# Tongji-MIC-Lab/TDVC

Measured on AMD Instinct MI355X. Metric: 1080p P-frames/sec (encode + reconstruct, lambda=2048 config), higher is better.
Workload: dtype f16; 1 GPU; 1x 1920x1080 (padded 1088x1920) 7-frame synthetic GOP (seed 1234), batch 1, P-frames coded in GOP order; gop=7, batch=1, parallelism=gop-sharded x1, weights=closed-form filler (no checkpoint ships)

## Files before the change

### include/tdvc_hip.h

```cpp
#ifndef TDVC_HIP_H
#define TDVC_HIP_H

#include <stdint.h>

#ifdef __cplusplus
extern "C" {
#endif

#define TDVC_OK 0
#define TDVC_EINVAL (-1)
#define TDVC_ENOSUP (-2)

typedef struct {
  void* p;
  int32_t N, H, W, C;
  int64_t sn;
  int32_t sp;
  int32_t dtype;
} tdvc_fmap;

enum { TDVC_F16 = 0, TDVC_F32 = 1 };
enum { TDVC_ACT_NONE = 0, TDVC_ACT_RELU = 1, TDVC_ACT_LRELU = 2, TDVC_ACT_CLAMP01 = 3, TDVC_ACT_SIGMOID = 4 };
enum { TDVC_GDN_NONE = 0, TDVC_GDN_FWD = 1, TDVC_GDN_INV = 2 };
enum { TDVC_OUT_NHWC = 0,
// ... 36 lines not shown
int tdvc_last_launch_predicated(void);
#define TDVC_MAX_PREDICATE_IMAGES 4
int tdvc_set_predicate_images(const int* flags, int n);
int tdvc_frame_changed(const tdvc_fmap* cur, tdvc_fmap* cache, int* flag, void* stream);
int tdvc_frames_changed(const tdvc_fmap* cur, tdvc_fmap* cache, int* flags, unsigned force_mask, void* stream);


int tdvc_conv_plan(int cin, int kh, int kw, int stride);
int64_t tdvc_conv_packed_bytes(int cout, int cin, int ntaps, int ck);
int tdvc_pack_conv_weights(const float* w_oihw, int cout, int cin_real, int cin, int kh, int kw,
                           int ntaps, const int8_t* tap_dy, const int8_t* tap_dx, int ck, uint16_t* dst);
int tdvc_conv2d(const tdvc_conv_desc* d, void* stream);
int tdvc_conv_chan_sum_rows(const tdvc_conv_desc* d);
int tdvc_conv_flow_supported(const tdvc_conv_desc* d);
const char* tdvc_conv_select(const tdvc_conv_desc* d);
int tdvc_conv2d_f32(const tdvc_conv_desc* d, void* stream);

typedef struct {
  tdvc_fmap x, y;
  const void* w;
  const float* bias;
  int32_t act1; float slope1;
  int32_t act2; float slope2;
  int32_t add_input;
  tdvc_fmap res2;
} tdvc_conv_pair_desc;
int64_t tdvc_conv_pair_packed_bytes(void);
int tdvc_pack_conv_pair_weights(const float* w1_oihw, const float* w2_oihw, uint16_t* dst);
int tdvc_conv_pair_supported(const tdvc_conv_pair_desc* d);
int tdvc_conv_pair(const tdvc_conv_pair_desc* d, void* stream);
// ... 256 lines not shown
```

### tdvc_amd/_lib.py

```python
from __future__ import annotations

import ctypes as C
import os

_HERE = os.path.dirname(os.path.abspath(__file__))
LIB_PATH = os.path.join(_HERE, "libtdvc_hip.so")

MAX_TAPS = 49
F16, F32 = 0, 1
ACT_NONE, ACT_RELU, ACT_LRELU, ACT_CLAMP01, ACT_SIGMOID = 0, 1, 2, 3, 4
GDN_NONE, GDN_FWD, GDN_INV = 0, 1, 2
OUT_NHWC, OUT_SHUFFLE2, OUT_NCHW_F32 = 0, 1, 2


class FMapDesc(C.Structure):
    _fields_ = [("p", C.c_void_p), ("N", C.c_int32), ("H", C.c_int32), ("W", C.c_int32), ("C", C.c_int32),
                ("sn", C.c_int64), ("sp", C.c_int32), ("dtype", C.c_int32)]


class ConvDesc(C.Structure):
    _fields_ = [("x", FMapDesc), ("y", FMapDesc), ("w", C.c_void_p), ("bias", C.c_void_p),
                ("cout", C.c_int32), ("ntaps", C.c_int32),
                ("tap_dy", C.c_int8 * MAX_TAPS), ("tap_dx", C.c_int8 * MAX_TAPS),
                ("kh", C.c_int32), ("kw", C.c_int32), ("stride", C.c_int32), ("pad", C.c_int32),
# ... 45 lines not shown

class LanesEncDesc(C.Structure):
    _fields_ = [("symbols", _P), ("indexes", _P), ("B", C.c_int32), ("H", C.c_int32), ("W", C.c_int32), ("M", C.c_int32), ("pos", _P),
                ("npos", C.c_int32), ("L", C.c_int32), ("scratch", _P), ("lane_words", C.c_int64), ("scratch_cap_words", C.c_int64),
                ("out", _P), ("out_stride", C.c_int64), ("out_cap", C.c_int64), ("info", _P)]


_LOOP, _CDF, _CDFD, _ENC = C.POINTER(ArLoopDesc), C.POINTER(CdfTablesDesc), C.POINTER(CdfTablesDevDesc), C.POINTER(LanesEncDesc)
_i, _f, _i64 = C.c_int, C.c_float, C.c_int64

SIGNATURES = {
    "tdvc_abi_version": (_i, []),
    "tdvc_conv_chan_sum_rows": (_i, [C.POINTER(ConvDesc)]),
    "tdvc_conv_select": (C.c_char_p, [C.POINTER(ConvDesc)]),
    "tdvc_conv_flow_supported": (_i, [C.POINTER(ConvDesc)]),
    "tdvc_scale_act_res3": (_i, [_FM, _P, _i, _f, _FM, _f, _FM, _FM, _f, _FM, _P]),
    "tdvc_avgpool2_pyramid": (_i, [_FM, _FM, _FM, _FM, _P]),
    "tdvc_last_error": (C.c_char_p, []),
    "tdvc_last_conv_kernel": (C.c_char_p, []),
    "tdvc_prepare_device": (_i, []),
    "tdvc_set_predicate": (_i, [_P]),
    "tdvc_set_predicate_images": (_i, [_P, _i]),
    "tdvc_last_launch_predicated": (_i, []),
    "tdvc_frame_changed": (_i, [_FM, _FM, _P, _P]),
    "tdvc_frames_changed": (_i, [_FM, _FM, _P, C.c_uint, _P]),
    "tdvc_conv_plan": (_i, [_i, _i, _i, _i]),
    "tdvc_conv_packed_bytes": (_i64, [_i, _i, _i, _i]),
    "tdvc_pack_conv_weights": (_i, [_P, _i, _i, _i, _i, _i, _i, _P, _P, _i, _P]),
    "tdvc_conv2d": (_i, [C.POINTER(ConvDesc), _P]),
    "tdvc_conv2d_f32": (_i, [C.POINTER(ConvDesc), _P]),
# ... 131 lines not shown
```

### tdvc_amd/csrc/conv_dispatch.hip

```cpp
#include <stdlib.h>

#include "conv_common.h"

using convk::ConvParams;
bool conv_v2_eligible(const tdvc_conv_desc* d, int Ho, int Wo); int launch_conv_v2(const ConvParams& p, int cout_blocks, int N, hipStream_t st);
bool conv_v3_eligible(const tdvc_conv_desc* d, int Ho, int Wo); int launch_conv_v3(const ConvParams& p, int cout_blocks, int N, hipStream_t st);
bool conv_v5_eligible(const tdvc_conv_desc* d, int Ho, int Wo); int launch_conv_v5(const ConvParams& p, int cout_blocks, int N, hipStream_t st); int conv_v5_chan_sum_rows(int Ho, int Wo, int cout_blocks, int N);
bool conv_v7_eligible(const tdvc_conv_desc* d, const ConvParams& p, int Ho, int Wo); int launch_conv_v7(const ConvParams& p, int cout_blocks, int N, hipStream_t st);
bool conv_v9_eligible(const tdvc_conv_desc* d, int Ho, int Wo, bool v3_ok); int launch_conv_v9(const ConvParams& p, int ck8, int cout_tiles32, int N, hipStream_t st);
bool conv_v10_eligible(const tdvc_conv_desc* d, const ConvParams& p, int Ho, int Wo); int launch_conv_v10(const ConvParams& p, int cout_blocks, int N, hipStream_t st);
bool conv_v11_eligible(const tdvc_conv_desc* d, const ConvParams& p, int Ho, int Wo); int launch_conv_v11(const ConvParams& p, int cout_blocks, int N, hipStream_t st);
int conv_row_geometry(const tdvc_conv_desc* d, const ConvParams& p, int Ho, int Wo); int launch_conv_row(int geo, const ConvParams& p, int N, hipStream_t st);
bool conv_c8_eligible(const tdvc_conv_desc* d, const ConvParams& p, int Ho, int Wo); int launch_conv_c8(const ConvParams& p, int N, hipStream_t st);
bool conv_n16_eligible(const tdvc_conv_desc* d, int Ho, int Wo); int launch_conv_n16(const ConvParams& p, int N, hipStream_t st);
bool gdn128_eligible(const tdvc_conv_desc* d, const ConvParams& p, int Ho, int Wo); int launch_gdn128(const ConvParams& p, int N, hipStream_t st);
int conv_direct_lds_bytes(const tdvc_conv_desc* d);
int conv_cout_tiles(int cout);
int launch_conv_direct(const ConvParams& p, int ck8, int stride, int N, hipStream_t st);
int conv_f32_validate(const tdvc_conv_desc* d, int& Ho, int& Wo);

namespace {
const char* const kSwitchEnv[convk::SW_COUNT] = {nullptr, "TDVC_CONV_NO_V3", "TDVC_CONV_NO_V5", "TDVC_CONV_NO_V7", "TDVC_CONV_NO_V9", "TDVC_CONV_NO_V10",
                                                 "TDVC_CONV_NO_V11", "TDVC_CONV_NO_ROW", "TDVC_CONV_NO_C8", "TDVC_CONV_NO_N16", "TDVC_CONV_NO_GDN128", "TDVC_CONV_NO_HEAD3"};
int g_enabled[convk::SW_COUNT] = {1, 1, 1, 1, 1, 1, 1, 15, 1, 1, 1, 1};
// ... 59 lines not shown
  return launch_conv_v5(q, 1, k.N(), st);
}
bool row_eligible(Pick& k, const ConvParams& p) { return (k.geo = conv_row_geometry(k.d, p, k.Ho, k.Wo)) >= 0; }

constexpr char kNameV5[] = "conv_mfma_v5", kNameDirect[] = "conv_mfma<%d,%d,%d>";

const Entry kTable[] = {
    {"conv_mfma_v5(bcast)", convk::SW_V5, bcast_eligible, bcast_launch, [](const tdvc_conv_desc* d) { return d->bcast_T != 0; },
     "tdvc_conv2d: bcast_T needs a plain 1x1 / stride 1 conv to 64 channels of >= 8192 pixels, y (and res, the optional source of the slices) a 64-channel window of a buffer with >= 4 slices, bcast_T == 4"},
    {"conv_row(s2d)", convk::SW_ROW, [](Pick& k, const ConvParams& p) { return k.d->s2d && row_eligible(k, p); },
     [](const Pick& k, const ConvParams& p, hipStream_t st) { return launch_conv_row(k.geo, p, k.N(), st); }, nullptr, nullptr},
    {"conv_mfma_v3(s2d)", convk::SW_V3, [](Pick& k, const ConvParams&) { return k.d->s2d && conv_v3_eligible(k.d, k.Ho, k.Wo); },
     [](const Pick& k, const ConvParams& p, hipStream_t st) { return launch_conv_v3(p, k.cout_blocks(), k.N(), st); },
     [](const tdvc_conv_desc* d) { return d->s2d != 0; }, "tdvc_conv2d: s2d conv not eligible for the stage-pipelined kernel"},
    {"conv_mfma_v9", convk::SW_V9, [](Pick& k, const ConvParams&) { return conv_v9_eligible(k.d, k.Ho, k.Wo, v3_on_and_eligible(k)); },
     [](const Pick& k, const ConvParams& p, hipStream_t st) { return launch_conv_v9(p, k.ck8(), conv_cout_tiles(k.d->cout), k.N(), st); }, nullptr, nullptr},
    {"gdn128", convk::SW_GDN128, [](Pick& k, const ConvParams& p) { return gdn128_eligible(k.d, p, k.Ho, k.Wo); },
     [](const Pick& k, const ConvParams& p, hipStream_t st) { return launch_gdn128(p, k.N(), st); }, nullptr, nullptr},
    {kNameV5, convk::SW_V5, [](Pick& k, const ConvParams&) { return conv_v5_eligible(k.d, k.Ho, k.Wo); },
     [](const Pick& k, const ConvParams& p, hipStream_t st) { return launch_conv_v5(p, k.cout_blocks(), k.N(), st); }, nullptr, nullptr},
    {"conv_c8", convk::SW_C8, [](Pick& k, const ConvParams& p) { return conv_c8_eligible(k.d, p, k.Ho, k.Wo); },
     [](const Pick& k, const ConvParams& p, hipStream_t st) { return launch_conv_c8(p, k.N(), st); }, nullptr, nullptr},
    {"conv_n16", convk::SW_N16, [](Pick& k, const ConvParams&) { return conv_n16_eligible(k.d, k.Ho, k.Wo); },
     [](const Pick& k, const ConvParams& p, hipStream_t st) { return launch_conv_n16(p, k.N(), st); }, nullptr, nullptr},
    {"conv_row", convk::SW_ROW, row_eligible,
     [](const Pick& k, const ConvParams& p, hipStream_t st) { return launch_conv_row(k.geo, p, k.N(), st); }, nullptr, nullptr},
    {"conv_mfma_v10", convk::SW_V10, [](Pick& k, const ConvParams& p) { return conv_v10_eligible(k.d, p, k.Ho, k.Wo); },
     [](const Pick& k, const ConvParams& p, hipStream_t st) { return launch_conv_v10(p, k.cout_blocks(), k.N(), st); }, nullptr, nullptr},
    {"conv_mfma_v7", convk::SW_V7, [](Pick& k, const ConvParams& p) { return conv_v7_eligible(k.d, p, k.Ho, k.Wo); },
     [](const Pick& k, const ConvParams& p, hipStream_t st) { return launch_conv_v7(p, k.cout_blocks(), k.N(), st); }, nullptr, nullptr},
    {"conv_mfma_v11", convk::SW_V11, [](Pick& k, const ConvParams& p) { return conv_v11_eligible(k.d, p, k.Ho, k.Wo); },
// ... 142 lines not shown
  p.csum = d->chan_sum;
  if (!e) return TDVC_EINVAL;
  if (d->flow.p) {
    TDVC_CHECK(conv_flow_ok(d, e, p) && flow_map_ok(d, k.Ho, k.Wo), "%s", kFlowMsg);
    p.flow = to_dev(d->flow);
  }
  kernel_name(e, k, g_last_kernel);
  return e->launch(k, p, reinterpret_cast<hipStream_t>(stream));
}

}

void tdvc_conv_walk_advance(int launches) { g_walk_parity += (unsigned)launches; }

extern "C" void tdvc_debug_set_conv_walk(int mode) { g_walk_mode = mode; }
extern "C" int tdvc_conv2d(const tdvc_conv_desc* d, void* stream) { return conv2d_impl(d, stream, LAUNCH); }
extern "C" int tdvc_conv_chan_sum_rows(const tdvc_conv_desc* d) { return conv2d_impl(d, nullptr, QUERY_ROWS); }
extern "C" int tdvc_conv_flow_supported(const tdvc_conv_desc* d) { return conv2d_impl(d, nullptr, QUERY_FLOW); }
extern "C" const char* tdvc_last_conv_kernel(void) { return g_last_kernel; }

extern "C" const char* tdvc_conv_select(const tdvc_conv_desc* d) {
  static thread_local char name[48];
  if (!d) { tdvc_set_error("tdvc_conv_select: null descriptor"); return nullptr; }
  if (d->x.dtype == TDVC_F32) {
    int Ho, Wo;
    if (d->flow.p) { tdvc_set_error("%s", kFlowMsg); return nullptr; }
    return conv_f32_validate(d, Ho, Wo) == TDVC_OK ? "conv_f32" : nullptr;
  }
  ConvParams p;
  Pick k = {d, 0, 0, -1};
  if (prepare(d, p, k.Ho, k.Wo) != TDVC_OK) return nullptr;
  const Entry* e = select(k, p);
  if (!e) return nullptr;
  if (d->flow.p && !(conv_flow_ok(d, e, p) && flow_map_ok(d, k.Ho, k.Wo))) { tdvc_set_error("%s", kFlowMsg); return nullptr; }
// ... 4 lines not shown
```

### tdvc_amd/csrc/conv_mfma_v9.hip

```cpp
#include "conv_common.h"

using convk::ConvParams;

namespace {

template <int CK8, int NW9>
__global__ __launch_bounds__(NW9 * 64) void conv_mfma_v9_kernel(const ConvParams p, int total_px) {
  __shared__ float red[NW9][32][33];
  __shared__ int tdy[TDVC_MAX_TAPS], tdx[TDVC_MAX_TAPS];
  constexpr int CK = CK8 * 8;
  const int tid = threadIdx.x, lane = tid & 63, wave = tid >> 6;
  const int hh = lane >> 5, r = lane & 31;
  const int ct = blockIdx.y;
  if (tid < p.ntaps) { tdy[tid] = p.tap_dy[tid]; tdx[tid] = p.tap_dx[tid]; }
  __syncthreads();

  const int px = blockIdx.x * 32 + r;
  const bool pv = px < total_px;
  const int pxc = pv ? px : 0;
  const int hw = p.Ho * p.Wo;
  const int n = pxc / hw, rem = pxc - n * hw;
  const int oy = rem / p.Wo, ox = rem - oy * p.Wo;
  const int iy0 = oy * p.in_stride - p.pad, ix0 = ox * p.in_stride - p.pad;
  const half_t* xn = p.x + (long)n * p.x_sn;

  const int T = p.nchunks * p.steps;
  const int g0 = (int)((long)T * wave / NW9), g1 = (int)((long)T * (wave + 1) / NW9);
  const half_t* wp = p.w + ((long)ct * T) * 512 + lane * 8;

  f32x16 acc;
#pragma unroll
  for (int i = 0; i < 16; ++i) acc[i] = 0.f;
  half8 zero8;
#pragma unroll
  for (int q = 0; q < 8; ++q) zero8[q] = (half_t)0.f;

  for (int g4 = g0; g4 < g1; g4 += 4) {
    half8 a[4], b[4];
    bool ok[4];
#pragma unroll
    for (int u = 0; u < 4; ++u) {
      const int g = min(g4 + u, g1 - 1);
      const int ch = g / p.steps, s = g - ch * p.steps;
      int tap, cofs;
      if constexpr (CK8 == 1) {
        tap = min(2 * s + hh, p.ntaps - 1);
        cofs = ch * 8;
      } else {
        constexpr int H2 = CK8 / 2;
        tap = s / H2;
        cofs = ch * CK + (s - tap * H2) * 16 + hh * 8;
      }
      const int iy = iy0 + tdy[tap], ix = ix0 + tdx[tap];
      ok[u] = pv && g4 + u < g1 && iy >= 0 && iy < p.H && ix >= 0 && ix < p.W && cofs < p.Cin;
      const int iyc = min(max(iy, 0), p.H - 1), ixc = min(max(ix, 0), p.W - 1), cc = min(cofs, p.Cin - 8);
      b[u] = *reinterpret_cast<const half8*>(xn + ((long)iyc * p.W + ixc) * p.x_sp + cc);
      a[u] = *reinterpret_cast<const half8*>(wp + (long)g * 512);
    }
#pragma unroll
    for (int u = 0; u < 4; ++u) {
      half8 bv = ok[u] ? b[u] : zero8;
      if (p.square) bv = bv * bv;
      acc = __builtin_amdgcn_mfma_f32_32x32x16_f16(a[u], bv, acc, 0, 0, 0);
    }
  }

#pragma unroll
  for (int i = 0; i < 16; ++i) red[wave][(i & 3) + 8 * (i >> 2) + 4 * hh][r] = acc[i];
  __syncthreads();
  for (int it = tid; it < 256; it += NW9 * 64) {
    const int pl = it & 31, grp = it >> 5;
    const int q = blockIdx.x * 32 + pl;
    if (q < total_px) {
      float v[4];
#pragma unroll
      for (int i = 0; i < 4; ++i) {
        float s = 0.f;
#pragma unroll
        for (int w = 0; w < NW9; ++w) s += red[w][4 * grp + i][pl];
        v[i] = s;
      }
      const int qn = q / hw, qr = q - qn * hw;
      const int qy = qr / p.Wo, qx = qr - qy * p.Wo;
      convk::epilogue4(p, qn, qy, qx, ct * 32 + 4 * grp, v);
    }
  }
}

}

bool conv_v9_eligible(const tdvc_conv_desc* d, int Ho, int Wo, bool v3_ok) {
  if (d->s2d) return false;
  const long px = (long)Ho * Wo * d->x.N;
  static const long maxpx = getenv("TDVC_V9_MAX_PX") ? atol(getenv("TDVC_V9_MAX_PX")) : convk::LARGE_MAP_PIXELS;
  static const long minpx = getenv("TDVC_V9_MIN_PX") ? atol(getenv("TDVC_V9_MIN_PX")) : 0;
  const long ksteps = (long)((d->x.C + d->ck - 1) / d->ck) * ((d->ntaps * (d->ck / 8) + 1) / 2);
  if (v3_ok && px * d->cout > convk::conv_v9_work_limit()) return false;
  return px <= maxpx && px >= minpx && ksteps >= 4 && (d->x.C % 8) == 0;
}

template <int CK8>
static void launch_v9_nw(const ConvParams& p, dim3 grid, int total, hipStream_t st) {
  const int T = p.nchunks * p.steps;
  if (T >= 32) hipLaunchKernelGGL((conv_mfma_v9_kernel<CK8, 8>), grid, dim3(512), 0, st, p, total);
  else if (T >= 16) hipLaunchKernelGGL((conv_mfma_v9_kernel<CK8, 4>), grid, dim3(256), 0, st, p, total);
  else if (T >= 8) hipLaunchKernelGGL((conv_mfma_v9_kernel<CK8, 2>), grid, dim3(128), 0, st, p, total);
  else hipLaunchKernelGGL((conv_mfma_v9_kernel<CK8, 1>), grid, dim3(64), 0, st, p, total);
}

int launch_conv_v9(const ConvParams& p, int ck8, int cout_tiles32, int N, hipStream_t st) {
  const int total = N * p.Ho * p.Wo;
  const dim3 grid((unsigned)((total + 31) / 32), (unsigned)cout_tiles32);
  switch (ck8) {
    case 1: launch_v9_nw<1>(p, grid, total, st); break;
    case 2: launch_v9_nw<2>(p, grid, total, st); break;
    case 4: launch_v9_nw<4>(p, grid, total, st); break;
    default: launch_v9_nw<8>(p, grid, total, st); break;
  }
  return tdvc_launch_status("tdvc_conv2d");
}
```

### tdvc_amd/csrc/lib.cpp

```cpp
#include <hip/hip_runtime.h>
#include <stdarg.h>
#include <stddef.h>
#include <stdio.h>

#include <mutex>

#include "../../include/tdvc_hip.h"

static thread_local char g_err[512] = "";

void tdvc_set_error(const char* fmt, ...) {
  va_list ap;
  va_start(ap, fmt);
  vsnprintf(g_err, sizeof(g_err), fmt, ap);
  va_end(ap);
}

static_assert(sizeof(tdvc_cdf_tables) == 32 && offsetof(tdvc_cdf_tables, ncdfs) == 28, "tdvc_cdf_tables layout");
static_assert(sizeof(tdvc_cdf_tables_dev) == 40 && offsetof(tdvc_cdf_tables_dev, ncdfs) == 36, "tdvc_cdf_tables_dev layout");
static_assert(sizeof(tdvc_ar_loop) == 272 && offsetof(tdvc_ar_loop, sym_dev) == 264, "tdvc_ar_loop layout");
static_assert(sizeof(tdvc_lf_tail_desc) == 168 && offsetof(tdvc_lf_tail_desc, slope) == 160, "tdvc_lf_tail_desc layout");
static_assert(sizeof(tdvc_lanes_enc) == 104 && offsetof(tdvc_lanes_enc, info) == 96, "tdvc_lanes_enc layout");

extern "C" int tdvc_abi_version(void) { return 16; }
extern "C" const char* tdvc_last_error(void) { return g_err; }

static thread_local const int* g_pred = nullptr;
static thread_local int g_pred_taken = 0, g_pred_last = 0;
static thread_local const int* g_pred_img = nullptr;
static thread_local int g_pred_img_n = 0;

extern "C" int tdvc_set_predicate(const int* flag) {
  if (reinterpret_cast<uintptr_t>(flag) & 3) { tdvc_set_error("tdvc_set_predicate: flag must be 4-byte aligned"); return TDVC_EINVAL; }
  if (flag && g_pred_img) { tdvc_set_error("tdvc_set_predicate: a per-image predicate is set (clear it first)"); return TDVC_EINVAL; }
  g_pred = flag;
  return TDVC_OK;
}
extern "C" int tdvc_set_predicate_images(const int* flags, int n) {
  if (!flags || n == 0) { g_pred_img = nullptr; g_pred_img_n = 0; return TDVC_OK; }
// ... 60 lines not shown
```

### tdvc_amd/model/coder.py

```python
from __future__ import annotations

import math
import threading

import numpy as np
import torch
import torch.nn as nn
import torch.nn.functional as F

from .. import ops
from ..ops import ACT_LRELU, ACT_NONE, FM, GDN_FWD, GDN_INV
from .modules import PackCache, SELayer, pk_conv


class _LowerBoundGrad(torch.autograd.Function):

    @staticmethod
    def forward(ctx, x, bound):
        ctx.save_for_backward(x, bound)
        return torch.max(x, bound)

    @staticmethod
    def backward(ctx, g):
        x, bound = ctx.saved_tensors
# ... 419 lines not shown
        t = ops.conv(t, pk_conv(self, "ep2", e[2]), **LR)
        return ops.conv(t, pk_conv(self, "ep4", e[4]), out_dtype=torch.float32)

    def ctx_conv(self) -> ops.PackedConv:
        cp = self.context_prediction

        def build():
            pc = ops.pack_conv(cp.weight, cp.bias, stride=1, pad=2, taps=cp.live_taps(), device=cp.weight.device)
            pc.orig["wgrad_taps"] = [(dy, dx) for dy in range(5) for dx in range(5)]
            return pc
        return self._pk("ctx", build)

    def _as_f32(self, x: FM) -> FM:
        return x if x.f32 else ops.cast_f32(x)

    def run(self, x: FM, training: bool, out: FM | None = None, res: FM | None = None, trace=None, noise=None, f32=False):
        dev = x.t.device
        xdt = torch.float32 if (f32 and x.f32) else torch.float16
        if f32:
            x = self._as_f32(x)
        adt = torch.float32 if f32 else torch.float16
        y32, y16 = self.run_g_a(x)
        z = self.run_h_a(y16)
        B, h, w, M = y32.N, y32.H, y32.W, self.M
        bits = torch.zeros(2, dtype=torch.float64, device=dev)
        z_hat = FM.empty(z.N, z.H, z.W, z.C, dtype=adt, device=dev)
        nz = ny = nl = None
        if training:
            noise = noise or {}
            nz = noise.get("z") or FM(torch.rand((z.N, z.H, z.W, z.C), device=dev) - 0.5)
            ny = noise.get("y") or FM(torch.rand((B, h, w, M), device=dev) - 0.5)
            nl = noise.get("y_lik") or FM(torch.rand((B, h, w, M), device=dev) - 0.5)
        ops.eb_forward(z, self.entropy_bottleneck.packed_params(), z_hat, bits[1:2], noise=nz)
        pcat = FM.empty(B, h, w, 4 * M, dtype=adt, device=dev)
        self.run_h_s(z_hat, out=pcat.ch(0, 2 * M))
        y_hat = ops.quantize(y32, FM.empty(B, h, w, M, dtype=adt, device=dev), noise=ny)
        ops.conv(y_hat, self.ctx_conv(), out=pcat.ch(2 * M, 2 * M))
        gp = self.run_entropy_parameters(pcat)
        ops.gc_forward(y32, gp, bits[0:1], noise=nl)
        x_hat = self.run_g_s(y_hat, out=out, res=res, out_dtype=xdt)
# ... 323 lines not shown
        sym = torch.zeros((g, H * W, M), dtype=torch.int32, device=dev)
        idx = torch.zeros((g, H * W, M), dtype=torch.int32, device=dev)
        if lanes:
            nl = ops.lanes_of(data[0])
            stream_dev = torch.empty(ops.ar_lanes_batch_layout([len(d) for d in data], nl)[0], dtype=torch.uint8, device=dev)
            try:
                ops.ar_wavefront_lanes_batch(lp, data, gct, stream_dev, ops.ar_lanes_state_batch(nl, g, dev), yh, pr, table, idx, sym)
            except ops.L.TdvcStreamError as e:
                raise ops.L.TdvcStreamError(f"decompress: image {members[e.image]} of the batch: corrupt or exhausted lane-split stream "
                                            "(a lane ran out of words or met an impossible code)") from None
        else:
            ops.ar_wavefront_batch(lp, data, gct, None, yh, pr, table, idx, sym)
        if scatter:
            y_hat_all.t[members] = yh.t

def _g_a(N):
    return nn.Sequential(
        ResidualBlockWithStride(64, N, stride=2), ResidualBlock(N, N),
        ResidualBlockWithStride(N, N, stride=2), SELayer(N), ResidualBlock(N, N),
        ResidualBlockWithStride(N, N, stride=2), ResidualBlock(N, N),
        conv3x3(N, N, stride=2), SELayer(N))


def _g_s(N):
    return nn.Sequential(
        SELayer(N), ResidualBlock(N, N), ResidualBlockUpsample(N, N, 2), ResidualBlock(N, N),
        ResidualBlockUpsample(N, N, 2), SELayer(N), ResidualBlock(N, N),
        ResidualBlockUpsample(N, N, 2), ResidualBlock(N, N), subpel_conv3x3(N, 64, 2))


# ... 13 lines not shown
```

### tdvc_amd/model/pnet.py

```python
from __future__ import annotations

import torch
import torch.nn as nn

from .. import ops
from ..ops import FM
from . import modules
from .coder import STREAM_CODERS, MVCoder, ResCoder
from .modules import FeaExtra, FeatureFix, LoopFilter, MCNet, OffsetGen


def _ref_views(refs8: FM, B: int):
    return (FM(refs8.t, refs8.off + 3 * refs8.sn, B, refs8.C, 4 * refs8.sn), FM(refs8.t, refs8.off, B, refs8.C, 4 * refs8.sn))


class VideoCompressor(nn.Module):
    fp32_islands_supported = True

    def __init__(self):
        super().__init__()
        self.coder_fp32 = False
        self.train_coder_fp32 = False
        self.model_fp32 = False
        self.train_model_fp32 = False
# ... 53 lines not shown
            refs8 = ops.from_nchw(refs, Cpad=8, dtype=adt)
            last = refer_frames[:, 3].float()
            ref32 = ops.from_nchw(last, Cpad=4, dtype=torch.float32)
            ref8, iframe8 = _ref_views(refs8, B)
            if ops.TAPE is not None:
                for t in (cur32, cur8, refs8, ref32, ref8, iframe8):
                    ops.TAPE.mark_input(t)

            feats = FM.empty(B, H, W, 192, dtype=adt, device=dev)
            npx_ = float(B * H * W)
            f_cur = self.extra_fea.run(cur8, feats.ch(0, 64))
            self.extra_fea.run(ref8, feats.ch(64, 64))
            estmv = self.motion_est.run(feats, cur32, ref32, traced=trace is not None or mf32)

            tr_mv = {} if trace is not None else None
            mv_hat, mv_bits = self.mvCoder.run(estmv, training=training, trace=tr_mv, noise=noise.get("mv"), f32=f32)
            coded = {}
            if is_compress:
                self.mvCoder.update(force=True)
                coded["mv"] = self.mvCoder.compress(estmv, f32=f32)

            xt = FM.empty(B, H, W, 256, dtype=adt, device=dev)
            pred1 = self.mcnet.run(mv_hat, feats, xt.ch(192, 64))
            pred = FM.empty(B, H, W, 64, dtype=adt, device=dev)
            resid = FM.empty(B, H, W, 64, dtype=adt, device=dev)
            if modules.RESID_FUSED and modules.glue_fusions_allowed(self, trace is not None or mf32):
                self.mcfilter.run(xt, refs8, pred, then=(f_cur, -1.0, resid))
            else:
                self.mcfilter.run(xt, refs8, pred)
                ops.scale_act_res(f_cur, resid, res=pred, res_sign=-1.0)

            tr_res = {} if trace is not None else None
            recon_f, res_bits = self.resCoder.run(resid, training=training, res=pred, trace=tr_res, noise=noise.get("res"), f32=f32)
            if is_compress:
                self.resCoder.update(force=True)
                coded["res"] = self.resCoder.compress(resid, f32=f32)
                self.last_strings = {k: v["strings"] for k, v in coded.items()}
                self.last_ac_bpp = {k: sum(len(s[0]) for s in v["strings"]) * 8.0 / npx_ for k, v in coded.items()}

            recon = self.loopfilter.run(recon_f, iframe8, training=training, trace=trace)

            npx = float(B * H * W)
            bpp_mv = (mv_bits.sum() / npx).float().view(-1)
            bpp_res = (res_bits.sum() / npx).float().view(-1)
            if trace is not None:
                trace.update(f_cur=f_cur, f_ref=feats.ch(64, 64), estmv=estmv, mv_x_hat=mv_hat, pred1=pred1, pred=pred,
                             resid=resid, recon_f=recon_f, mv=tr_mv, res=tr_res)
        if training:
# ... 138 lines not shown
```

### tdvc_amd/ops.py

```python
from __future__ import annotations

import ctypes as C
from dataclasses import dataclass

import numpy as np
import torch

from . import _lib as L
from . import convpack
from ._lib import (ACT_CLAMP01, ACT_LRELU, ACT_NONE, ACT_RELU, GDN_FWD, GDN_INV, GDN_NONE, OUT_NCHW_F32,
                   OUT_NHWC, OUT_SHUFFLE2)


_raw_stream = torch._C._cuda_getCurrentRawStream
_cur_dev = torch._C._cuda_getDevice
FORCE_STREAM = None
FORCE_KEEP = None


def _stream():
    if FORCE_STREAM is not None:
        return C.c_void_p(FORCE_STREAM)
    return C.c_void_p(_raw_stream(_cur_dev()))

# ... 476 lines not shown
        e1.record()
        PROFILE.append(dict(kernel=L.lib().tdvc_last_conv_kernel().decode(),
                            shape=f"{pc.kh}x{pc.kw} s{pc.stride} {x.C}->{pc.cout} @{x.H}x{x.W}" + (" f32out" if out_dtype == torch.float32 else "") + (" nchw" if nchw_out is not None else ""),
                            e0=e0, e1=e1,
                            flops=2.0 * x.N * Ho * Wo * pc.cout * x.C * len(pc.taps),
                            flops_real=(x.N * Ho * Wo * pc.flops_per_px) if pc.s2d else 2.0 * x.N * Ho * Wo * pc.cout * pc.cin_real * len(pc.taps),
                            bytes=2.0 * x.N * (x.H * x.W * x.C + Ho * Wo * pc.cout * (4 if pc.shuffle else 1) / (4 if pc.shuffle else 1))))
        _rec("conv", x, rec_pc, None if nchw_out is not None else ret, act, slope, res, res2, gdn, aux, square, nchw_out)
        return ret
    L.check(L.lib().tdvc_conv2d(C.byref(d), _stream()), "conv2d")
    _log_predicated()
    _rec("conv", x, rec_pc, None if nchw_out is not None else ret, act, slope, res, res2, gdn, aux, square, nchw_out)
    return ret


class rgb_head_kernel:

    def __init__(self, enable: bool):
        self.enable = bool(enable)

    def __enter__(self):
        if not self.enable:
            L.lib().tdvc_debug_enable_conv_head3(0)
        return self

    def __exit__(self, *exc):
        if not self.enable:
            L.lib().tdvc_debug_enable_conv_head3(1)
        return False

# ... 1027 lines not shown
```

Measured before the change: 52.58 frames/s.

## Batch mv and residual hyperprior rate paths into paired v9 conv launches with register tiling

Defers the mv coder's hyperprior and entropy-parameter rate path so it runs together with the residual coder's identical-geometry path. Each layer pair goes out as one conv_mfma_v9 launch with a z-dimension of two problems, falling back to two launches when unsupported. The v9 kernel also gains multi-tile register blocking (MT x NT output tiles per workgroup, picked from grid size), so weight and input loads are reused across several tiles. These target launch count and underfilled grids on the small latent-resolution convs, at the cost of more registers, more template instantiations and a reordered schedule between the two coders.

```diff
diff --git a/include/tdvc_hip.h b/include/tdvc_hip.h
--- a/include/tdvc_hip.h
+++ b/include/tdvc_hip.h
@@ -74,6 +74,12 @@
 int tdvc_conv_chan_sum_rows(const tdvc_conv_desc* d);
 int tdvc_conv_flow_supported(const tdvc_conv_desc* d);
 const char* tdvc_conv_select(const tdvc_conv_desc* d);
+int tdvc_conv_v9_form(const tdvc_conv_desc* d);
+int tdvc_debug_set_conv_v9_form(int mt, int nt);
+int tdvc_debug_conv_v9_last_form(void);
+int tdvc_conv2d_pair2_supported(const tdvc_conv_desc* a, const tdvc_conv_desc* b);
+unsigned tdvc_debug_conv_walk_parity(void);
+int tdvc_conv2d_pair2(const tdvc_conv_desc* a, const tdvc_conv_desc* b, void* stream);
 int tdvc_conv2d_f32(const tdvc_conv_desc* d, void* stream);
 
 typedef struct {
diff --git a/tdvc_amd/_lib.py b/tdvc_amd/_lib.py
--- a/tdvc_amd/_lib.py
+++ b/tdvc_amd/_lib.py
@@ -7,6 +7,7 @@
 LIB_PATH = os.path.join(_HERE, "libtdvc_hip.so")
 
 MAX_TAPS = 49
+ENOSUP = -2
 F16, F32 = 0, 1
 ACT_NONE, ACT_RELU, ACT_LRELU, ACT_CLAMP01, ACT_SIGMOID = 0, 1, 2, 3, 4
 GDN_NONE, GDN_FWD, GDN_INV = 0, 1, 2
@@ -83,6 +84,12 @@
     "tdvc_conv_chan_sum_rows": (_i, [C.POINTER(ConvDesc)]),
     "tdvc_conv_select": (C.c_char_p, [C.POINTER(ConvDesc)]),
     "tdvc_conv_flow_supported": (_i, [C.POINTER(ConvDesc)]),
+    "tdvc_conv_v9_form": (_i, [C.POINTER(ConvDesc)]),
+    "tdvc_debug_set_conv_v9_form": (_i, [_i, _i]),
+    "tdvc_debug_conv_v9_last_form": (_i, []),
+    "tdvc_conv2d_pair2_supported": (_i, [C.POINTER(ConvDesc), C.POINTER(ConvDesc)]),
+    "tdvc_debug_conv_walk_parity": (C.c_uint, []),
+    "tdvc_conv2d_pair2": (_i, [C.POINTER(ConvDesc), C.POINTER(ConvDesc), _P]),
     "tdvc_scale_act_res3": (_i, [_FM, _P, _i, _f, _FM, _f, _FM, _FM, _f, _FM, _P]),
     "tdvc_avgpool2_pyramid": (_i, [_FM, _FM, _FM, _FM, _P]),
     "tdvc_last_error": (C.c_char_p, []),
diff --git a/tdvc_amd/csrc/conv_dispatch.hip b/tdvc_amd/csrc/conv_dispatch.hip
--- a/tdvc_amd/csrc/conv_dispatch.hip
+++ b/tdvc_amd/csrc/conv_dispatch.hip
@@ -7,7 +7,7 @@
 bool conv_v3_eligible(const tdvc_conv_desc* d, int Ho, int Wo); int launch_conv_v3(const ConvParams& p, int cout_blocks, int N, hipStream_t st);
 bool conv_v5_eligible(const tdvc_conv_desc* d, int Ho, int Wo); int launch_conv_v5(const ConvParams& p, int cout_blocks, int N, hipStream_t st); int conv_v5_chan_sum_rows(int Ho, int Wo, int cout_blocks, int N);
 bool conv_v7_eligible(const tdvc_conv_desc* d, const ConvParams& p, int Ho, int Wo); int launch_conv_v7(const ConvParams& p, int cout_blocks, int N, hipStream_t st);
-bool conv_v9_eligible(const tdvc_conv_desc* d, int Ho, int Wo, bool v3_ok); int launch_conv_v9(const ConvParams& p, int ck8, int cout_tiles32, int N, hipStream_t st);
+bool conv_v9_eligible(const tdvc_conv_desc* d, int Ho, int Wo, bool v3_ok); int launch_conv_v9(const ConvParams& p, const ConvParams* pb, int ck8, int cout_tiles32, int N, hipStream_t st); int conv_v9_pick_form(int px_tiles, int cout_tiles, int T);
 bool conv_v10_eligible(const tdvc_conv_desc* d, const ConvParams& p, int Ho, int Wo); int launch_conv_v10(const ConvParams& p, int cout_blocks, int N, hipStream_t st);
 bool conv_v11_eligible(const tdvc_conv_desc* d, const ConvParams& p, int Ho, int Wo); int launch_conv_v11(const ConvParams& p, int cout_blocks, int N, hipStream_t st);
 int conv_row_geometry(const tdvc_conv_desc* d, const ConvParams& p, int Ho, int Wo); int launch_conv_row(int geo, const ConvParams& p, int N, hipStream_t st);
@@ -97,7 +97,7 @@
      [](const Pick& k, const ConvParams& p, hipStream_t st) { return launch_conv_v3(p, k.cout_blocks(), k.N(), st); },
      [](const tdvc_conv_desc* d) { return d->s2d != 0; }, "tdvc_conv2d: s2d conv not eligible for the stage-pipelined kernel"},
     {"conv_mfma_v9", convk::SW_V9, [](Pick& k, const ConvParams&) { return conv_v9_eligible(k.d, k.Ho, k.Wo, v3_on_and_eligible(k)); },
-     [](const Pick& k, const ConvParams& p, hipStream_t st) { return launch_conv_v9(p, k.ck8(), conv_cout_tiles(k.d->cout), k.N(), st); }, nullptr, nullptr},
+     [](const Pick& k, const ConvParams& p, hipStream_t st) { return launch_conv_v9(p, nullptr, k.ck8(), conv_cout_tiles(k.d->cout), k.N(), st); }, nullptr, nullptr},
     {"gdn128", convk::SW_GDN128, [](Pick& k, const ConvParams& p) { return gdn128_eligible(k.d, p, k.Ho, k.Wo); },
      [](const Pick& k, const ConvParams& p, hipStream_t st) { return launch_gdn128(p, k.N(), st); }, nullptr, nullptr},
     {kNameV5, convk::SW_V5, [](Pick& k, const ConvParams&) { return conv_v5_eligible(k.d, k.Ho, k.Wo); },
@@ -270,10 +270,53 @@
 void tdvc_conv_walk_advance(int launches) { g_walk_parity += (unsigned)launches; }
 
 extern "C" void tdvc_debug_set_conv_walk(int mode) { g_walk_mode = mode; }
+extern "C" unsigned tdvc_debug_conv_walk_parity(void) { return g_walk_parity; }
 extern "C" int tdvc_conv2d(const tdvc_conv_desc* d, void* stream) { return conv2d_impl(d, stream, LAUNCH); }
 extern "C" int tdvc_conv_chan_sum_rows(const tdvc_conv_desc* d) { return conv2d_impl(d, nullptr, QUERY_ROWS); }
 extern "C" int tdvc_conv_flow_supported(const tdvc_conv_desc* d) { return conv2d_impl(d, nullptr, QUERY_FLOW); }
 extern "C" const char* tdvc_last_conv_kernel(void) { return g_last_kernel; }
+
+namespace {
+const Entry* select_v9(const tdvc_conv_desc* d, ConvParams& p, Pick& k) {
+  if (!d || d->x.dtype == TDVC_F32 || d->chan_sum || d->flow.p) return nullptr;
+  if (prepare(d, p, k.Ho, k.Wo) != TDVC_OK) return nullptr;
+  const Entry* e = select(k, p);
+  return e && e->sw == convk::SW_V9 ? e : nullptr;
+}
+bool same_v9_geometry(const tdvc_conv_desc* a, const tdvc_conv_desc* b) {
+  return a->x.N == b->x.N && a->x.H == b->x.H && a->x.W == b->x.W && a->x.C == b->x.C && a->cout == b->cout && a->ntaps == b->ntaps &&
+         a->kh == b->kh && a->kw == b->kw && a->stride == b->stride && a->pad == b->pad && a->ck == b->ck &&
+         memcmp(a->tap_dy, b->tap_dy, a->ntaps) == 0 && memcmp(a->tap_dx, b->tap_dx, a->ntaps) == 0;
+}
+}
+
+extern "C" int tdvc_conv_v9_form(const tdvc_conv_desc* d) {
+  if (!d) { tdvc_set_error("tdvc_conv_v9_form: null descriptor"); return TDVC_EINVAL; }
+  if (!tdvc_conv_select(d)) return TDVC_EINVAL;
+  ConvParams p;
+  Pick k = {d, 0, 0, -1};
+  if (!select_v9(d, p, k)) return 0;
+  return conv_v9_pick_form((int)(((long)k.N() * k.Ho * k.Wo + 31) / 32), conv_cout_tiles(d->cout), p.nchunks * p.steps);
+}
+
+extern "C" int tdvc_conv2d_pair2_supported(const tdvc_conv_desc* a, const tdvc_conv_desc* b) {
+  ConvParams pa, pb;
+  Pick ka = {a, 0, 0, -1}, kb = {b, 0, 0, -1};
+  return select_v9(a, pa, ka) && select_v9(b, pb, kb) && same_v9_geometry(a, b) ? 1 : 0;
+}
+
+extern "C" int tdvc_conv2d_pair2(const tdvc_conv_desc* a, const tdvc_conv_desc* b, void* stream) {
+  ConvParams pa, pb;
+  Pick ka = {a, 0, 0, -1}, kb = {b, 0, 0, -1};
+  if (!(select_v9(a, pa, ka) && select_v9(b, pb, kb) && same_v9_geometry(a, b))) {
+    tdvc_set_error("tdvc_conv2d_pair2: needs two descriptors of one geometry that tdvc_conv_select sends to conv_mfma_v9 (tdvc_conv2d_pair2_supported() == 0)");
+    return TDVC_ENOSUP;
+  }
+  pa.reverse = next_walk_reverse();
+  pb.reverse = next_walk_reverse();
+  snprintf(g_last_kernel, sizeof(g_last_kernel), "conv_mfma_v9");
+  return launch_conv_v9(pa, &pb, ka.ck8(), conv_cout_tiles(a->cout), ka.N(), reinterpret_cast<hipStream_t>(stream));
+}
 
 extern "C" const char* tdvc_conv_select(const tdvc_conv_desc* d) {
   static thread_local char name[48];
diff --git a/tdvc_amd/csrc/conv_mfma_v9.hip b/tdvc_amd/csrc/conv_mfma_v9.hip
--- a/tdvc_amd/csrc/conv_mfma_v9.hip
+++ b/tdvc_amd/csrc/conv_mfma_v9.hip
@@ -4,40 +4,50 @@
 
 namespace {
 
-template <int CK8, int NW9>
-__global__ __launch_bounds__(NW9 * 64) void conv_mfma_v9_kernel(const ConvParams p, int total_px) {
-  __shared__ float red[NW9][32][33];
-  __shared__ int tdy[TDVC_MAX_TAPS], tdx[TDVC_MAX_TAPS];
+template <int CK8, int NW9, int MT, int NT>
+__device__ __forceinline__ void conv_v9_body(const ConvParams& p, int total_px, int cout_tiles, float (&red)[NW9][32][33], int* tdy, int* tdx) {
   constexpr int CK = CK8 * 8;
   const int tid = threadIdx.x, lane = tid & 63, wave = tid >> 6;
   const int hh = lane >> 5, r = lane & 31;
-  const int ct = blockIdx.y;
   if (tid < p.ntaps) { tdy[tid] = p.tap_dy[tid]; tdx[tid] = p.tap_dx[tid]; }
   __syncthreads();
 
-  const int px = blockIdx.x * 32 + r;
-  const bool pv = px < total_px;
-  const int pxc = pv ? px : 0;
   const int hw = p.Ho * p.Wo;
-  const int n = pxc / hw, rem = pxc - n * hw;
-  const int oy = rem / p.Wo, ox = rem - oy * p.Wo;
-  const int iy0 = oy * p.in_stride - p.pad, ix0 = ox * p.in_stride - p.pad;
-  const half_t* xn = p.x + (long)n * p.x_sn;
-
   const int T = p.nchunks * p.steps;
   const int g0 = (int)((long)T * wave / NW9), g1 = (int)((long)T * (wave + 1) / NW9);
-  const half_t* wp = p.w + ((long)ct * T) * 512 + lane * 8;
-
-  f32x16 acc;
-#pragma unroll
-  for (int i = 0; i < 16; ++i) acc[i] = 0.f;
+
+  bool pv[NT];
+  int iy0[NT], ix0[NT];
+  const half_t* xn[NT];
+#pragma unroll
+  for (int j = 0; j < NT; ++j) {
+    const int px = (blockIdx.x * NT + j) * 32 + r;
+    pv[j] = px < total_px;
+    const int pxc = pv[j] ? px : 0;
+    const int n = pxc / hw, rem = pxc - n * hw;
+    const int oy = rem / p.Wo, ox = rem - oy * p.Wo;
+    iy0[j] = oy * p.in_stride - p.pad;
+    ix0[j] = ox * p.in_stride - p.pad;
+    xn[j] = p.x + (long)n * p.x_sn;
+  }
+  const half_t* wp[MT];
+#pragma unroll
+  for (int i = 0; i < MT; ++i) wp[i] = p.w + ((long)min((int)blockIdx.y * MT + i, cout_tiles - 1) * T) * 512 + lane * 8;
+
+  f32x16 acc[MT][NT];
+#pragma unroll
+  for (int i = 0; i < MT; ++i)
+#pragma unroll
+    for (int j = 0; j < NT; ++j)
+#pragma unroll
+      for (int e = 0; e < 16; ++e) acc[i][j][e] = 0.f;
   half8 zero8;
 #pragma unroll
   for (int q = 0; q < 8; ++q) zero8[q] = (half_t)0.f;
 
   for (int g4 = g0; g4 < g1; g4 += 4) {
-    half8 a[4], b[4];
-    bool ok[4];
+    half8 a[4][MT], b[4][NT];
+    bool ok[4][NT];
 #pragma unroll
     for (int u = 0; u < 4; ++u) {
       const int g = min(g4 + u, g1 - 1);
@@ -51,40 +61,78 @@
         tap = s / H2;
         cofs = ch * CK + (s - tap * H2) * 16 + hh * 8;
       }
-      const int iy = iy0 + tdy[tap], ix = ix0 + tdx[tap];
-      ok[u] = pv && g4 + u < g1 && iy >= 0 && iy < p.H && ix >= 0 && ix < p.W && cofs < p.Cin;
-      const int iyc = min(max(iy, 0), p.H - 1), ixc = min(max(ix, 0), p.W - 1), cc = min(cofs, p.Cin - 8);
-      b[u] = *reinterpret_cast<const half8*>(xn + ((long)iyc * p.W + ixc) * p.x_sp + cc);
-      a[u] = *reinterpret_cast<const half8*>(wp + (long)g * 512);
+      const int cc = min(cofs, p.Cin - 8);
+#pragma unroll
+      for (int j = 0; j < NT; ++j) {
+        const int iy = iy0[j] + tdy[tap], ix = ix0[j] + tdx[tap];
+        ok[u][j] = pv[j] && g4 + u < g1 && iy >= 0 && iy < p.H && ix >= 0 && ix < p.W && cofs < p.Cin;
+        const int iyc = min(max(iy, 0), p.H - 1), ixc = min(max(ix, 0), p.W - 1);
+        b[u][j] = *reinterpret_cast<const half8*>(xn[j] + ((long)iyc * p.W + ixc) * p.x_sp + cc);
+      }
+#pragma unroll
+      for (int i = 0; i < MT; ++i) a[u][i] = *reinterpret_cast<const half8*>(wp[i] + (long)g * 512);
     }
 #pragma unroll
     for (int u = 0; u < 4; ++u) {
-      half8 bv = ok[u] ? b[u] : zero8;
-      if (p.square) bv = bv * bv;
-      acc = __builtin_amdgcn_mfma_f32_32x32x16_f16(a[u], bv, acc, 0, 0, 0);
+      half8 bv[NT];
+#pragma unroll
+      for (int j = 0; j < NT; ++j) {
+        bv[j] = ok[u][j] ? b[u][j] : zero8;
+        if (p.square) bv[j] = bv[j] * bv[j];
+      }
+#pragma unroll
+      for (int i = 0; i < MT; ++i)
+#pragma unroll
+        for (int j = 0; j < NT; ++j) acc[i][j] = __builtin_amdgcn_mfma_f32_32x32x16_f16(a[u][i], bv[j], acc[i][j], 0, 0, 0);
     }
   }
 
 #pragma unroll
-  for (int i = 0; i < 16; ++i) red[wave][(i & 3) + 8 * (i >> 2) + 4 * hh][r] = acc[i];
-  __syncthreads();
-  for (int it = tid; it < 256; it += NW9 * 64) {
-    const int pl = it & 31, grp = it >> 5;
-    const int q = blockIdx.x * 32 + pl;
-    if (q < total_px) {
-      float v[4];
-#pragma unroll
-      for (int i = 0; i < 4; ++i) {
-        float s = 0.f;
-#pragma unroll
-        for (int w = 0; w < NW9; ++w) s += red[w][4 * grp + i][pl];
-        v[i] = s;
-      }
-      const int qn = q / hw, qr = q - qn * hw;
-      const int qy = qr / p.Wo, qx = qr - qy * p.Wo;
-      convk::epilogue4(p, qn, qy, qx, ct * 32 + 4 * grp, v);
+  for (int i = 0; i < MT; ++i) {
+#pragma unroll
+    for (int j = 0; j < NT; ++j) {
+      const int ct = blockIdx.y * MT + i, pt = blockIdx.x * NT + j;
+      if (i + j > 0) {
+        if (ct >= cout_tiles || pt * 32 >= total_px) continue;
+        __syncthreads();
+      }
+#pragma unroll
+      for (int e = 0; e < 16; ++e) red[wave][(e & 3) + 8 * (e >> 2) + 4 * hh][r] = acc[i][j][e];
+      __syncthreads();
+      for (int it = tid; it < 256; it += NW9 * 64) {
+        const int pl = it & 31, grp = it >> 5;
+        const int q = pt * 32 + pl;
+        if (q < total_px) {
+          float v[4];
+#pragma unroll
+          for (int e = 0; e < 4; ++e) {
+            float s = 0.f;
+#pragma unroll
+            for (int w = 0; w < NW9; ++w) s += red[w][4 * grp + e][pl];
+            v[e] = s;
+          }
+          const int qn = q / hw, qr = q - qn * hw;
+          const int qy = qr / p.Wo, qx = qr - qy * p.Wo;
+          convk::epilogue4(p, qn, qy, qx, ct * 32 + 4 * grp, v);
+        }
+      }
     }
   }
+}
+
+template <int CK8, int NW9, int MT, int NT>
+__global__ __launch_bounds__(NW9 * 64) void conv_mfma_v9_kernel(const ConvParams p, int total_px, int cout_tiles) {
+  __shared__ float red[NW9][32][33];
+  __shared__ int tdy[TDVC_MAX_TAPS], tdx[TDVC_MAX_TAPS];
+  conv_v9_body<CK8, NW9, MT, NT>(p, total_px, cout_tiles, red, tdy, tdx);
+}
+
+template <int CK8, int NW9, int MT, int NT>
+__global__ __launch_bounds__(NW9 * 64) void conv_mfma_v9_pair_kernel(const ConvParams pa, const ConvParams pb, int total_px, int cout_tiles) {
+  __shared__ float red[NW9][32][33];
+  __shared__ int tdy[TDVC_MAX_TAPS], tdx[TDVC_MAX_TAPS];
+  if (blockIdx.z == 0) conv_v9_body<CK8, NW9, MT, NT>(pa, total_px, cout_tiles, red, tdy, tdx);
+  else conv_v9_body<CK8, NW9, MT, NT>(pb, total_px, cout_tiles, red, tdy, tdx);
 }
 
 }
@@ -99,23 +147,71 @@
   return px <= maxpx && px >= minpx && ksteps >= 4 && (d->x.C % 8) == 0;
 }
 
+namespace {
+int g_v9_forced_form = 0;
+thread_local int g_v9_last_form = 0;
+constexpr int V9_FORMS[] = {0x202, 0x201, 0x102, 0x401, 0x101};
+constexpr int V9_WGS_2X2 = 512, V9_WGS_2X1 = 384, V9_PX_TILES_4X1 = 192;
+}
+
+int conv_v9_pick_form(int px_tiles, int cout_tiles, int T) {
+  (void)T;
+  const long P = px_tiles, Ct = cout_tiles;
+  if (P >= 2 && Ct >= 2 && ((P + 1) / 2) * ((Ct + 1) / 2) >= V9_WGS_2X2) return 0x202;
+  if (Ct == 4 && P >= V9_PX_TILES_4X1) return 0x401;
+  if (Ct >= 2 && P * ((Ct + 1) / 2) >= V9_WGS_2X1) return 0x201;
+  return 0x101;
+}
+
+extern "C" int tdvc_debug_set_conv_v9_form(int mt, int nt) {
+  const int f = (mt << 8) | nt;
+  if (mt == 0 && nt == 0) { g_v9_forced_form = 0; return TDVC_OK; }
+  for (const int c : V9_FORMS)
+    if (c == f) { g_v9_forced_form = f; return TDVC_OK; }
+  tdvc_set_error("tdvc_debug_set_conv_v9_form: no form <%d, %d> (1x1, 2x1, 1x2, 2x2, 4x1; 0, 0 = automatic)", mt, nt);
+  return TDVC_EINVAL;
+}
+extern "C" int tdvc_debug_conv_v9_last_form(void) { return g_v9_last_form; }
+
+template <int CK8, int NW9, int MT, int NT>
+static void launch_v9_form(const ConvParams& pa, const ConvParams& pb, int nproblems, int total, int cout_tiles, hipStream_t st) {
+  const int px_tiles = (total + 31) / 32;
+  const dim3 grid((unsigned)((px_tiles + NT - 1) / NT), (unsigned)((cout_tiles + MT - 1) / MT), (unsigned)nproblems);
+  if (nproblems == 2) hipLaunchKernelGGL((conv_mfma_v9_pair_kernel<CK8, NW9, MT, NT>), grid, dim3(NW9 * 64), 0, st, pa, pb, total, cout_tiles);
+  else hipLaunchKernelGGL((conv_mfma_v9_kernel<CK8, NW9, MT, NT>), grid, dim3(NW9 * 64), 0, st, pa, total, cout_tiles);
+}
+
+template <int CK8, int NW9>
+static void launch_v9_forms(int form, const ConvParams& pa, const ConvParams& pb, int nproblems, int total, int cout_tiles, hipStream_t st) {
+  switch (form) {
+    case 0x202: launch_v9_form<CK8, NW9, 2, 2>(pa, pb, nproblems, total, cout_tiles, st); break;
+    case 0x201: launch_v9_form<CK8, NW9, 2, 1>(pa, pb, nproblems, total, cout_tiles, st); break;
+    case 0x102: launch_v9_form<CK8, NW9, 1, 2>(pa, pb, nproblems, total, cout_tiles, st); break;
+    case 0x401: launch_v9_form<CK8, NW9, 4, 1>(pa, pb, nproblems, total, cout_tiles, st); break;
+    default: launch_v9_form<CK8, NW9, 1, 1>(pa, pb, nproblems, total, cout_tiles, st); break;
+  }
+}
+
 template <int CK8>
-static void launch_v9_nw(const ConvParams& p, dim3 grid, int total, hipStream_t st) {
-  const int T = p.nchunks * p.steps;
-  if (T >= 32) hipLaunchKernelGGL((conv_mfma_v9_kernel<CK8, 8>), grid, dim3(512), 0, st, p, total);
-  else if (T >= 16) hipLaunchKernelGGL((conv_mfma_v9_kernel<CK8, 4>), grid, dim3(256), 0, st, p, total);
-  else if (T >= 8) hipLaunchKernelGGL((conv_mfma_v9_kernel<CK8, 2>), grid, dim3(128), 0, st, p, total);
-  else hipLaunchKernelGGL((conv_mfma_v9_kernel<CK8, 1>), grid, dim3(64), 0, st, p, total);
-}
-
-int launch_conv_v9(const ConvParams& p, int ck8, int cout_tiles32, int N, hipStream_t st) {
+static void launch_v9_nw(int form, const ConvParams& pa, const ConvParams& pb, int nproblems, int total, int cout_tiles, hipStream_t st) {
+  const int T = pa.nchunks * pa.steps;
+  if (T >= 32) launch_v9_forms<CK8, 8>(form, pa, pb, nproblems, total, cout_tiles, st);
+  else if (T >= 16) launch_v9_forms<CK8, 4>(form, pa, pb, nproblems, total, cout_tiles, st);
+  else if (T >= 8) launch_v9_forms<CK8, 2>(form, pa, pb, nproblems, total, cout_tiles, st);
+  else launch_v9_forms<CK8, 1>(form, pa, pb, nproblems, total, cout_tiles, st);
+}
+
+int launch_conv_v9(const ConvParams& p, const ConvParams* pb, int ck8, int cout_tiles32, int N, hipStream_t st) {
   const int total = N * p.Ho * p.Wo;
-  const dim3 grid((unsigned)((total + 31) / 32), (unsigned)cout_tiles32);
+  const int form = g_v9_forced_form ? g_v9_forced_form : conv_v9_pick_form((total + 31) / 32, cout_tiles32, p.nchunks * p.steps);
+  g_v9_last_form = form;
+  const ConvParams& q = pb ? *pb : p;
+  const int np = pb ? 2 : 1;
   switch (ck8) {
-    case 1: launch_v9_nw<1>(p, grid, total, st); break;
-    case 2: launch_v9_nw<2>(p, grid, total, st); break;
-    case 4: launch_v9_nw<4>(p, grid, total, st); break;
-    default: launch_v9_nw<8>(p, grid, total, st); break;
+    case 1: launch_v9_nw<1>(form, p, q, np, total, cout_tiles32, st); break;
+    case 2: launch_v9_nw<2>(form, p, q, np, total, cout_tiles32, st); break;
+    case 4: launch_v9_nw<4>(form, p, q, np, total, cout_tiles32, st); break;
+    default: launch_v9_nw<8>(form, p, q, np, total, cout_tiles32, st); break;
   }
   return tdvc_launch_status("tdvc_conv2d");
 }
diff --git a/tdvc_amd/csrc/lib.cpp b/tdvc_amd/csrc/lib.cpp
--- a/tdvc_amd/csrc/lib.cpp
+++ b/tdvc_amd/csrc/lib.cpp
@@ -22,7 +22,7 @@
 static_assert(sizeof(tdvc_lf_tail_desc) == 168 && offsetof(tdvc_lf_tail_desc, slope) == 160, "tdvc_lf_tail_desc layout");
 static_assert(sizeof(tdvc_lanes_enc) == 104 && offsetof(tdvc_lanes_enc, info) == 96, "tdvc_lanes_enc layout");
 
-extern "C" int tdvc_abi_version(void) { return 16; }
+extern "C" int tdvc_abi_version(void) { return 17; }
 extern "C" const char* tdvc_last_error(void) { return g_err; }
 
 static thread_local const int* g_pred = nullptr;
diff --git a/tdvc_amd/model/coder.py b/tdvc_amd/model/coder.py
--- a/tdvc_amd/model/coder.py
+++ b/tdvc_amd/model/coder.py
@@ -457,16 +457,26 @@
     def _as_f32(self, x: FM) -> FM:
         return x if x.f32 else ops.cast_f32(x)
 
-    def run(self, x: FM, training: bool, out: FM | None = None, res: FM | None = None, trace=None, noise=None, f32=False):
+    def run(self, x: FM, training: bool, out: FM | None = None, res: FM | None = None, trace=None, noise=None, f32=False,
+            defer_rate: list | None = None, paired_rate: list | None = None):
         dev = x.t.device
         xdt = torch.float32 if (f32 and x.f32) else torch.float16
         if f32:
             x = self._as_f32(x)
         adt = torch.float32 if f32 else torch.float16
         y32, y16 = self.run_g_a(x)
-        z = self.run_h_a(y16)
         B, h, w, M = y32.N, y32.H, y32.W, self.M
         bits = torch.zeros(2, dtype=torch.float64, device=dev)
+        if defer_rate is not None or paired_rate:
+            assert not training and trace is None and not f32
+            y_hat = ops.quantize(y32, FM.empty(B, h, w, M, dtype=adt, device=dev))
+            mine = (self, y32, y16, y_hat, bits)
+            if defer_rate is not None:
+                defer_rate.append(mine)
+            else:
+                rate_paths_paired(paired_rate.pop(), mine)
+            return self.run_g_s(y_hat, out=out, res=res, out_dtype=xdt), bits
+        z = self.run_h_a(y16)
         z_hat = FM.empty(z.N, z.H, z.W, z.C, dtype=adt, device=dev)
         nz = ny = nl = None
         if training:
@@ -820,6 +830,44 @@
         if scatter:
             y_hat_all.t[members] = yh.t
 
+RATE_PAIRED = True
+
+
+def rate_paths_paired(a, b) -> None:
+    (ca, y32a, ta, yha, bits_a), (cb, y32b, tb, yhb, bits_b) = a, b
+    assert (y32a.N, y32a.H, y32a.W, ca.M) == (y32b.N, y32b.H, y32b.W, cb.M)
+    dev, f32 = y32a.t.device, torch.float32
+    B, h, w, M = y32a.N, y32a.H, y32a.W, ca.M
+
+    def pair(xa, xb, key, layer, kwa=None, kwb=None, **kw):
+        pca, pcb = (pk_conv(c, key, layer(c)) if key else layer(c) for c in (ca, cb))
+        return ops.conv2((xa, pca, dict(kw, **(kwa or {}))), (xb, pcb, dict(kw, **(kwb or {}))))
+    for i in (0, 2, 4, 6):
+        ta, tb = pair(ta, tb, f"ha{i}", lambda c, i=i: c.h_a[i], **LR)
+    za, zb = pair(ta, tb, "ha8", lambda c: c.h_a[8], out_dtype=f32)
+    zs = []
+    for c, z, bits in ((ca, za, bits_a), (cb, zb, bits_b)):
+        z_hat = FM.empty(z.N, z.H, z.W, z.C, device=dev)
+        ops.eb_forward(z, c.entropy_bottleneck.packed_params(), z_hat, bits[1:2])
+        zs.append(z_hat)
+    pa, pb = (FM.empty(B, h, w, 4 * M, device=dev) for _ in range(2))
+    ta, tb = pair(zs[0], zs[1], "hs0", lambda c: c.h_s[0], **LR)
+    ta, tb = _pair_shuffle(ca, cb, ta, tb, "hs2", 2)
+    ta, tb = pair(ta, tb, "hs4", lambda c: c.h_s[4], **LR)
+    ta, tb = _pair_shuffle(ca, cb, ta, tb, "hs6", 6)
+    pair(ta, tb, "hs8", lambda c: c.h_s[8], kwa=dict(out=pa.ch(0, 2 * M)), kwb=dict(out=pb.ch(0, 2 * M)))
+    pair(yha, yhb, None, lambda c: c.ctx_conv(), kwa=dict(out=pa.ch(2 * M, 2 * M)), kwb=dict(out=pb.ch(2 * M, 2 * M)))
+    ta, tb = pair(pa, pb, "ep0", lambda c: c.entropy_parameters[0], **LR)
+    ta, tb = pair(ta, tb, "ep2", lambda c: c.entropy_parameters[2], **LR)
+    ga, gb = pair(ta, tb, "ep4", lambda c: c.entropy_parameters[4], out_dtype=f32)
+    ops.gc_forward(y32a, ga, bits_a[0:1])
+    ops.gc_forward(y32b, gb, bits_b[0:1])
+
+
+def _pair_shuffle(ca, cb, ta, tb, key, i):
+    return ops.conv2((ta, pk_conv(ca, key, ca.h_s[i][0], shuffle=True), dict(LR)), (tb, pk_conv(cb, key, cb.h_s[i][0], shuffle=True), dict(LR)))
+
+
 def _g_a(N):
     return nn.Sequential(
         ResidualBlockWithStride(64, N, stride=2), ResidualBlock(N, N),
diff --git a/tdvc_amd/model/pnet.py b/tdvc_amd/model/pnet.py
--- a/tdvc_amd/model/pnet.py
+++ b/tdvc_amd/model/pnet.py
@@ -6,6 +6,7 @@
 from .. import ops
 from ..ops import FM
 from . import modules
+from . import coder as coder_mod
 from .coder import STREAM_CODERS, MVCoder, ResCoder
 from .modules import FeaExtra, FeatureFix, LoopFilter, MCNet, OffsetGen
 
@@ -91,7 +92,8 @@
             estmv = self.motion_est.run(feats, cur32, ref32, traced=trace is not None or mf32)
 
             tr_mv = {} if trace is not None else None
-            mv_hat, mv_bits = self.mvCoder.run(estmv, training=training, trace=tr_mv, noise=noise.get("mv"), f32=f32)
+            rate = [] if (coder_mod.RATE_PAIRED and not f32 and not is_compress and modules.glue_fusions_allowed(self, trace is not None or mf32)) else None
+            mv_hat, mv_bits = self.mvCoder.run(estmv, training=training, trace=tr_mv, noise=noise.get("mv"), f32=f32, defer_rate=rate)
             coded = {}
             if is_compress:
                 self.mvCoder.update(force=True)
@@ -108,7 +110,7 @@
                 ops.scale_act_res(f_cur, resid, res=pred, res_sign=-1.0)
 
             tr_res = {} if trace is not None else None
-            recon_f, res_bits = self.resCoder.run(resid, training=training, res=pred, trace=tr_res, noise=noise.get("res"), f32=f32)
+            recon_f, res_bits = self.resCoder.run(resid, training=training, res=pred, trace=tr_res, noise=noise.get("res"), f32=f32, paired_rate=rate)
             if is_compress:
                 self.resCoder.update(force=True)
                 coded["res"] = self.resCoder.compress(resid, f32=f32)
diff --git a/tdvc_amd/ops.py b/tdvc_amd/ops.py
--- a/tdvc_amd/ops.py
+++ b/tdvc_amd/ops.py
@@ -514,6 +514,22 @@
     return ret
 
 
+def conv2(a: tuple, b: tuple) -> tuple:
+    if TAPE is not None or PROFILE is not None:
+        raise L.TdvcHipError("conv2: inference only (under the tape or the per-kernel profile call conv twice)")
+    (xa, pca, kwa), (xb, pcb, kwb) = a, b
+    da, ra = conv_desc(xa, pca, **kwa)[:2]
+    db, rb = conv_desc(xb, pcb, **kwb)[:2]
+    rc = L.lib().tdvc_conv2d_pair2(C.byref(da), C.byref(db), _stream())
+    if rc == L.ENOSUP:
+        L.check(L.lib().tdvc_conv2d(C.byref(da), _stream()), "conv2d")
+        L.check(L.lib().tdvc_conv2d(C.byref(db), _stream()), "conv2d")
+    else:
+        L.check(rc, "conv2d_pair2")
+    _log_predicated(2)
+    return ra, rb
+
+
 class rgb_head_kernel:
 
     def __init__(self, enable: bool):
```

New measurement: 52.60 frames/s (median of 2 runs). Within noise of the previous version (+0.0%).
